# ubc-vision/DiffuseSG

Hardware: NVIDIA B200
Metric: sampled scene graphs/sec (higher is better)
Workload: dtype bf16

## Files before the change

### diffusesg_b200/build_native.py

```python
from __future__ import annotations

import os
import subprocess
import sys
from concurrent.futures import ThreadPoolExecutor

HERE = os.path.dirname(os.path.abspath(__file__))
CSRC = os.path.join(HERE, "csrc")
LIB_DIR = os.path.join(HERE, "lib")
LIB_PATH = os.path.join(LIB_DIR, "libdsg_b200.so")
SOURCES = ["gemm.cu", "mlp.cu", "blocktail.cu", "blockhead.cu", "projln.cu", "attention.cu", "attention_tc.cu", "rowops.cu", "edm.cu", "train.cu", "backward.cu", "pack.cu", "model.cu"]
HEADERS = ["common.cuh", "kernels.h", os.path.join("..", "..", "include", "dsg_b200.h")]
NVCC_FLAGS = ["-gencode", "arch=compute_100a,code=sm_100a", "-lineinfo", "-O3", "-std=c++17",
              "-Xcompiler", "-fPIC", "-Xcompiler", "-fvisibility=hidden", "--expt-relaxed-constexpr"]


def _nvcc() -> str:
    for cand in (os.environ.get("NVCC"), "/usr/local/cuda/bin/nvcc", "nvcc"):
        if cand and (os.path.isabs(cand) and os.path.exists(cand) or not os.path.isabs(cand)):
            return cand
    raise RuntimeError("nvcc not found")


def _stale(target: str, deps) -> bool:
    if not os.path.exists(target):
        return True
    t = os.path.getmtime(target)
    return any(os.path.getmtime(d) > t for d in deps)


def build(force: bool = False, verbose: bool = False) -> str:
    os.makedirs(LIB_DIR, exist_ok=True)
    hdrs = [os.path.normpath(os.path.join(CSRC, h)) for h in HEADERS]
    objs, jobs = [], []
    for src in SOURCES:
        s = os.path.join(CSRC, src)
        o = os.path.join(LIB_DIR, src.replace(".cu", ".o"))
        objs.append(o)
        if force or _stale(o, [s] + hdrs):
            jobs.append([_nvcc(), *NVCC_FLAGS, *(["-Xptxas", "-v"] if verbose else []), "-c", s, "-o", o])

    def run(cmd):
        r = subprocess.run(cmd, capture_output=True, text=True)
        if r.returncode != 0:
            raise RuntimeError("nvcc failed: %s\n%s\n%s" % (" ".join(cmd), r.stdout, r.stderr))
        return r.stderr

    with ThreadPoolExecutor(max_workers=6) as ex:
        for out in ex.map(run, jobs):
            if verbose and out:
                print(out)
    if force or jobs or _stale(LIB_PATH, objs):
        run([_nvcc(), "-shared", "-o", LIB_PATH, *objs, "-lcudart"])
    return LIB_PATH


if __name__ == "__main__":
    print(build(force="--force" in sys.argv, verbose="-v" in sys.argv))
```

### diffusesg_b200/csrc/blocktail.cu

```cuda
#include "common.cuh"
#include "kernels.h"

namespace dsg {
namespace {

constexpr int kTailThreads = 19 * 32;
constexpr float kTailLnEps = 1e-5f;

template <int C>
struct TailCfg {
  static constexpr int HID = 4 * C;
  static constexpr int HC = 128;
  static constexpr int NCH = HID / HC;
  static constexpr int KBN = C / 32;
  static constexpr int A_KB = 128 * 64;
  static constexpr int A_BYTES = KBN * A_KB;
  static constexpr int W1_KB = HC * 64;
  static constexpr int W1_SLOT = KBN * W1_KB;
  static constexpr int WP_KB = C * 64;
  static constexpr int W2_KB = C * 128;
  static constexpr int W2_SLOT = (HC / 64) * W2_KB;
  static constexpr int S1 = 2, S2 = 2;
  static constexpr int XB = C / 32;
  static constexpr int X_BYTES = XB * 16384;
// ... 472 lines not shown
        return;
      }
      if (tl > 0) mbar_wait(out_free, (tl - 1) & 1);
#pragma unroll
      for (int i = 0; i < G::CW; i += 4)
        *reinterpret_cast<float4*>(sXo + ((c0 + i) >> 5) * 16384 + r_t * 128 + ((((((c0 + i) & 31) >> 2)) ^ (r_t & 7)) << 4)) =
            make_float4(__uint_as_float(v[i]), __uint_as_float(v[i + 1]), __uint_as_float(v[i + 2]), __uint_as_float(v[i + 3]));
      fence_proxy_async_smem();
      __syncwarp();
      if (lane == 0) mbar_arrive(out_ready);
    };

    auto phase_g = [&](int g) {
      const int b = g & 1, j = g % G::NCH;
      mbar_wait(&acc1_full[b], (g >> 1) & 1);
      tcgen05_fence_after();
#pragma unroll
      for (int h = 0; h < 2; ++h) {
        const int col = cg * 32 + h * 16;
        uint32_t r[16];
        tmem_ld_32x16(t_lane + b * G::HC + col, r);
        tmem_ld_wait();
        uint32_t hp[8];
#pragma unroll
        for (int k = 0; k < 16; k += 4) {
          const float4 bb = *reinterpret_cast<const float4*>(&sB1[j * G::HC + col + k]);
          hp[k >> 1] = gelu_bias_bf16x2(r[k], r[k + 1], bb.x, bb.y);
          hp[(k >> 1) + 1] = gelu_bias_bf16x2(r[k + 2], r[k + 3], bb.z, bb.w);
        }
        tmem_st_32x8(t_lane + b * G::HC + col, hp);
      }
      tmem_st_wait();
      tcgen05_fence_before();
      __syncwarp();
      if (lane == 0) mbar_arrive(&h_full[b]);
    };

    if (my_tiles > 0) phase_p(0);
    for (int tl = 0; tl < my_tiles; ++tl) {
      const int g0 = tl * G::NCH;
      phase_g(g0);
      if (tl > 0) phase_o(tl - 1);
#pragma unroll 1
      for (int j = 1; j < G::NCH - 1; ++j) phase_g(g0 + j);
      if (tl + 1 < my_tiles) {
        mbar_wait(&acc1_full[(g0 + G::NCH - 1) & 1], ((g0 + G::NCH - 1) >> 1) & 1);
        phase_p(tl + 1);
      }
      phase_g(g0 + G::NCH - 1);
    }
    if (my_tiles > 0) phase_o(my_tiles - 1);
  }

  tcgen05_fence_before();
  __syncthreads();
  tcgen05_fence_after();
  if (warp == kMmaWarp) tmem_dealloc<512>(tmem_base);
}

template <int C>
int launch_c(const CUtensorMap* tmAtt, const CUtensorMap* tmWp, const CUtensorMap* tmW1, const CUtensorMap* tmW2,
             const CUtensorMap* tmX, const CUtensorMap* tmY, const TailParams& p, cudaStream_t st) {
  static PerDeviceOnce configured;
  if (configured.first()) {
    DSG_CUDA_CHECK(cudaFuncSetAttribute(block_tail_kernel<C, false>, cudaFuncAttributeMaxDynamicSharedMemorySize,
                                        TailCfg<C>::SMEM_BYTES));
    DSG_CUDA_CHECK(cudaFuncSetAttribute(block_tail_kernel<C, true>, cudaFuncAttributeMaxDynamicSharedMemorySize,
                                        TailCfg<C>::SMEM_BYTES));
  }
  const int sms = device_sm_count();
  const int tiles = (p.M + 127) / 128;
  if (tmY != nullptr)
    block_tail_kernel<C, true><<<tiles < sms ? tiles : sms, kTailThreads, TailCfg<C>::SMEM_BYTES, st>>>(
        *tmAtt, *tmWp, *tmW1, *tmW2, *tmX, *tmY, p);
  else
    block_tail_kernel<C, false><<<tiles < sms ? tiles : sms, kTailThreads, TailCfg<C>::SMEM_BYTES, st>>>(
        *tmAtt, *tmWp, *tmW1, *tmW2, *tmX, *tmX, p);
  DSG_LAUNCH_CHECK();
  return DSG_OK;
}

}

bool block_tail_supported(int C) { return C == 96; }

int launch_block_tail(const CUtensorMap* tmAtt, const CUtensorMap* tmWp, const CUtensorMap* tmW1,
                      const CUtensorMap* tmW2, const CUtensorMap* tmX, const float* bp, const float* gamma,
                      const float* beta, const float* b1, const float* b2, float* x, long long rows, int C,
                      cudaStream_t st, const CUtensorMap* tmY, const float* gamma_f, const float* beta_f) {
  DSG_REQUIRE(block_tail_supported(C) && rows > 0 && rows < 2147483647LL, "block_tail: C=%d rows=%lld", C, rows);
  DSG_REQUIRE((tmY == nullptr) == (gamma_f == nullptr) && (tmY == nullptr) == (beta_f == nullptr),
              "block_tail: the fused final LayerNorm needs its output map, gamma and beta together");
  TailParams p{bp, gamma, beta, b1, b2, x, gamma_f, beta_f, static_cast<int>(rows)};
  return launch_c<96>(tmAtt, tmWp, tmW1, tmW2, tmX, tmY, p, st);
}

}
```

### diffusesg_b200/csrc/kernels.h

```cpp
#pragma once

#include <cuda.h>
#include <cuda_bf16.h>
#include <cuda_runtime.h>
#include <stdint.h>

namespace dsg {

typedef __nv_bfloat16 bf16;

enum GemmEpi : int {
  EPI_BF16 = 0,
  EPI_GELU_BF16 = 1,
  EPI_RES_F32 = 2,
  EPI_F32 = 3,
  EPI_ADJ_HEAD = 4,
};

struct GemmParams {
  int M, N, K;
  const float* bias;
  const float* res;
  void* out;
  int ldo;
  int bn;
  int ksplit;
  int scale_rows;
  float row_scale;
  const float* w2t;
  const float* b2;
  int c_e;
  int n_img;
  const uint8_t* flags;
  const float* x_adj;
  const float* c_skip;
  const float* c_out;
  const int* perm;
  int side;
};

int make_tmap_bf16(CUtensorMap* map, const void* base, int64_t rows, int64_t cols, int box_rows);
int make_tmap_out(CUtensorMap* map, const void* base, int64_t rows, int64_t cols, int epi);

int launch_wgrad(const void* dy, const void* x, float* dw, long long tokens, int n_out, int x_cols, int out_cols, int ksplit,
                 int scale_rows, float row_scale, cudaStream_t st);

int gemm_block_n(int N);
int gemm_choose_bn(long long rows, int N, int K, int epi, bool pair);
bool gemm_use_pair(long long rows, int K, int epi);
int launch_gemm(const CUtensorMap* tmA, const CUtensorMap* tmW, const CUtensorMap* tmO, int epi, const GemmParams& p,
                cudaStream_t st, bool pair = false);

bool fused_mlp_supported(int C);
int fused_mlp_w1_box_rows(int C);
int launch_fused_mlp(const CUtensorMap* tmY, const CUtensorMap* tmW1, const CUtensorMap* tmW2, const CUtensorMap* tmX,
                     const float* b1, const float* b2, long long rows, int C, cudaStream_t st);

int make_tmap_2d(CUtensorMap* map, const void* base, int64_t rows, int64_t cols, int elem_bytes, int box_cols,
                 int box_rows);
bool block_tail_supported(int C);
int launch_block_tail(const CUtensorMap* tmAtt, const CUtensorMap* tmWp, const CUtensorMap* tmW1,
                      const CUtensorMap* tmW2, const CUtensorMap* tmX, const float* bp, const float* gamma,
                      const float* beta, const float* b1, const float* b2, float* x, long long rows, int C,
                      cudaStream_t st, const CUtensorMap* tmY = nullptr,
                      const float* gamma_f = nullptr, const float* beta_f = nullptr);

bool proj_ln_supported(int C);
int launch_proj_ln(const CUtensorMap* tmA, const CUtensorMap* tmW, const float* bias, const float* gamma, const float* beta,
                   float* x, bf16* y, long long rows, int C, cudaStream_t st);

bool block_head_supported(int C);
int launch_block_head(const CUtensorMap* tmXin, const CUtensorMap* tmXout, const CUtensorMap* tmW, const CUtensorMap* tmQ,
                      const float* film, int film_ld, int cond_uniform, int tokens_per_sample, const float* gamma,
                      const float* beta, const float* bqkv, long long rows, int C, cudaStream_t st);

int make_tmap_3d_bf16(CUtensorMap* map, const void* base, int64_t d0, int64_t d1, int64_t d2, int64_t s1, int64_t s2, int b0,
                      int b1, int b2);
bool window_attention_tc_supported(int batch, int res, int window, int shift, int heads);
int launch_window_attention_tc(const bf16* qkv, const float* bias, bf16* out, int batch, int res, int shift, int heads,
                               cudaStream_t st);
int launch_window_attention_tc_groups(const bf16* qkv, const float* bias, bf16* out, int n_groups, const int* counts,
                                      const int* res, const long long* tok_off, int heads, cudaStream_t st);
bool window_attention_quad_supported(int batch, int res, int window, int shift, int heads);
int launch_window_attention_quad(const bf16* qkv, const float* bias, bf16* out, int batch, int res, int window, int shift,
                                 int heads, cudaStream_t st);
int check_mask_canonical(const float* mask, int res, int window, int shift, cudaStream_t st, int* canonical);
bool window_attention_w16_supported(int batch, int res, int window, int shift, int heads);
int launch_window_attention_w16(const bf16* qkv, const float* bias, bf16* out, int batch, int res, int shift, int heads,
                                cudaStream_t st);
int check_bias_toeplitz(const float* bias, int heads, int window, cudaStream_t st, int* toeplitz);
enum { ATTN_MASK_CANONICAL = 1, ATTN_BIAS_TOEPLITZ = 2 };
int launch_window_attention(const bf16* qkv, const float* bias, const float* mask, bf16* out, int batch, int res,
                            int window, int shift, int heads, cudaStream_t st, int canonical = 0);

int launch_film_ln(const float* x_in, float* x_out, bf16* y, const float* film, int film_ld, int film_off,
                   int cond_uniform, const float* gamma, const float* beta, int batch, int tokens_per_sample,
                   int C, cudaStream_t st, const int* src_rows = nullptr);
int launch_ln(const float* x, bf16* y, const float* gamma, const float* beta, int64_t rows, int C, cudaStream_t st);
int launch_merge_ln(const float* x, bf16* y, const float* gamma, const float* beta, int batch, int res, int C,
                    cudaStream_t st);
int launch_concat_bf16(const float* x, const float* skip, bf16* y, int64_t rows, int C, cudaStream_t st,
                       const int* skip_rows = nullptr);
int launch_breakup_ln(const float* t, bf16* y, const float* g1, const float* b1, const float* g2, const float* b2,
                      int batch, int res, int D, cudaStream_t st);

int launch_cond(const float* noise_labels, long long label_stride, int n_cond, const float* w0, const float* b0, const float* w1,
                const float* b1, const float* w_film, const float* b_film, int film_total, float* emb0, float* emb1,
                float* emb, float* film, int embed, cudaStream_t st);

int launch_precond_coef(const float* sigmas, int sigma_stride, float* coef, int batch, cudaStream_t st);

int launch_node_proj(const float* node, const float* sc_node, const float* in_scale, const float* w_rc,
                     float* rc, int batch, int n, int c_n, int self_cond, int embed, cudaStream_t st);
int launch_patch_embed(const float* adj, const float* sc_adj, const float* in_scale, const uint8_t* flags,
                       const float* rc, const float* w_adj, const float* bias, const float* gamma,
                       const float* beta, const float* film, int film_ld, int film_off, int cond_uniform,
                       float* x0, int batch, int n, int c_e, int self_cond, int embed, cudaStream_t st,
                       const int* perm = nullptr, int side = 0);
int launch_node_head(const bf16* rep, const uint8_t* flags, const float* fold_t, const float* fold_b, const float* w1t,
                     const float* b1, const float* w2t, const float* b2, const float* x_node, const float* c_skip, const float* c_out,
                     float* out_node, int batch, int n, int c_n, int embed, cudaStream_t st, const int* tok0 = nullptr,
                     const int* width = nullptr, float* scratch = nullptr);

bool row_compaction_supported(int C_merge, int D_breakup);
int launch_breakup_ln_compact(const float* t, bf16* y, const float* g1, const float* b1, const float* g2, const float* b2,
                              int batch, int res, int D, const int* tok0, const int* width, int sh, cudaStream_t st,
                              const int* src_perm = nullptr);


int launch_edm_pre_step(const float* adj, const float* node, const float* eps_adj, const float* eps_node,
                        const uint8_t* flags, float noise_coef, float* adj_hat, float* node_hat, int batch,
                        int c_e, int n, int c_n, cudaStream_t st);
int launch_edm_pre_step_philox(const float* adj, const float* node, const uint8_t* flags, float noise_coef,
                               unsigned long long seed, unsigned long long offset_adj, int grid_adj,
                               unsigned long long offset_node, int grid_node, const void* dev_params, float* adj_hat,
                               float* node_hat, int batch, int c_e, int n, int c_n, cudaStream_t st);
int launch_edm_post_step(const float* adj_hat, const float* node_hat, const float* d1_adj, const float* d1_node,
                         const float* d2_adj, const float* d2_node, const uint8_t* flags, float inv_t_hat,
                         float h, float inv_t_prime, const void* dev_params, float* adj_next, float* node_next, int batch,
                         int c_e, int n, int c_n, cudaStream_t st);
int launch_edm_step_advance(const void* table, void* cur, int* counter, cudaStream_t st);
int launch_edm_final_decode(const float* adj_hat, const float* node_hat, const float* d1_adj, const float* d1_node,
                            const uint8_t* flags, float inv_t_hat, float h, const void* dev_params, float* adj_next,
                            float* node_next, int32_t* adj_cls, int32_t* node_cls, float* bbox, int num_adj_type,
                            int num_node_type, int batch, int c_e, int n, int c_n, cudaStream_t st);
int launch_mask_scale(const float* adj, const float* node, const uint8_t* flags, float scale, float* adj_out,
                      float* node_out, int batch, int c_e, int n, int c_n, cudaStream_t st);

// ... 25 lines not shown
```

### diffusesg_b200/csrc/model.cu

```cuda
#include <cstdarg>
#include <cstdio>
#include <cstdlib>
#include <cstring>
#include <map>
#include <string>
#include <tuple>
#include <vector>

#include "../../include/dsg_b200.h"
#include "common.cuh"
#include "kernels.h"

namespace dsg {

static thread_local char g_err[1024] = "";
static unsigned long long g_launches = 0;
static int g_stop_after = -1;

void set_last_error(const char* fmt, ...) {
  va_list ap;
  va_start(ap, fmt);
  vsnprintf(g_err, sizeof(g_err), fmt, ap);
  va_end(ap);
}
// ... 436 lines not shown
  p.M = static_cast<int>(rows); p.N = W.N; p.K = W.K;
  p.bias = bias; p.res = res; p.out = out; p.ldo = W.N;
  const double mn = static_cast<double>(rows) * W.N;
  const double out_bytes = epi == EPI_ADJ_HEAD ? static_cast<double>(rows) * (extra ? extra->c_e : 0) * 4
                                               : mn * ((epi == EPI_BF16 || epi == EPI_GELU_BF16) ? 2 : 4);
  char label[56];
  snprintf(label, sizeof(label), "gemm_n%d_k%d_epi%d", W.N, W.K, epi);
  ProfScope ps(g_prof_pass, PC_GEMM, 2.0 * mn * W.K,
               static_cast<double>(rows) * W.K * 2 + static_cast<double>(W.N) * W.K * 2 + out_bytes +
                   (epi == EPI_RES_F32 ? mn * 4 : 0), st, label, rows, W.K);
  const bool pair = gemm_use_pair(rows, W.K, epi);
  p.bn = gemm_choose_bn(rows, W.N, W.K, epi, pair);
  if (p.bn == 256) return launch_gemm(&it->second, pair ? &W.tmap256_half : &W.tmap256, tmo, epi, p, st, pair);
  return launch_gemm(&it->second, pair ? &W.tmap_half : &W.tmap, tmo, epi, p, st, pair);
}

#define DSG_TRY(expr)        \
  do {                       \
    int _rc = (expr);        \
    if (_rc) return _rc;     \
  } while (0)

#define DSG_TRY_P(cls, flops, bytes, expr)                                    \
  do {                                                                        \
    ProfScope _ps(g_prof_pass, cls, flops, bytes, st, #expr);                 \
    int _rc = (expr);                                                         \
    if (_rc) return _rc;                                                      \
  } while (0)

int run_block(dsg_model* m, const Block& b, const Workspace& w, const float* x_in, int batch, int cond_uniform,
              cudaStream_t st, bool fuse_final_ln = false, bool* fused_final_ln = nullptr, const Compact* cp = nullptr,
              const int* x_in_rows = nullptr) {
  const int C = b.dim;
  const int L = b.res * b.res;
  const long long rows = cp != nullptr ? cp->tokens(b.stage) : static_cast<long long>(batch) * L;
  const std::string& p = b.prefix;
  const double rc = static_cast<double>(rows) * C;
  auto tmap = [&](const void* ptr, int key, auto make) -> const CUtensorMap* {
    auto k = std::make_tuple(ptr, rows, key);
    auto it = m->a_maps.find(k);
    if (it == m->a_maps.end()) {
      CUtensorMap tm;
      if (make(&tm)) return nullptr;
      it = m->a_maps.emplace(k, tm).first;
    }
    return &it->second;
  };
  DSG_REQUIRE(x_in_rows == nullptr || (x_in != w.X && !block_head_supported(C)), "run_block: layout-changing input at C = %d", C);
  if (m->use_head && block_head_supported(C)) {
    const CUtensorMap* ti = tmap(x_in, -(C * 8 + EPI_RES_F32), [&](CUtensorMap* t) { return make_tmap_out(t, x_in, rows, C, EPI_RES_F32); });
    const CUtensorMap* to = tmap(w.X, -(C * 8 + EPI_RES_F32), [&](CUtensorMap* t) { return make_tmap_out(t, w.X, rows, C, EPI_RES_F32); });
    const CUtensorMap* tq = tmap(w.QKV, -(3 * C * 8 + EPI_BF16), [&](CUtensorMap* t) { return make_tmap_out(t, w.QKV, rows, 3 * C, EPI_BF16); });
    if (ti == nullptr || to == nullptr || tq == nullptr) return DSG_ERR_CUDA;
    DSG_TRY_P(PC_MLP, 6.0 * rc * C, rc * 14,
              launch_block_head(ti, to, &b.head_w, tq, w.film + b.film_off, m->film_total, cond_uniform, L,
                                m->f32(p + ".norm1.weight"), m->f32(p + ".norm1.bias"), m->at<float>(b.qkv_bias_off), rows,
                                C, st));
  } else {
    DSG_TRY_P(PC_ROW, 0, rc * 10, launch_film_ln(x_in, w.X, w.Y, w.film, m->film_total, b.film_off, cond_uniform,
                                                 m->f32(p + ".norm1.weight"), m->f32(p + ".norm1.bias"),
                                                 cp != nullptr ? 1 : batch, cp != nullptr ? static_cast<int>(rows) : L, C, st,
                                                 x_in_rows));
    DSG_TRY(gemm(m, w.Y, rows, b.qkv, EPI_BF16, m->at<float>(b.qkv_bias_off), nullptr, w.QKV, st));
  }
  const float* mask = b.shift > 0 ? m->f32(p + ".attn_mask") : nullptr;
  if (cp != nullptr && b.window == 8 && cp->K <= 4) {
    int res_k[4];
    long long tok_k[4];
    for (int k = 0; k < cp->K; ++k) { res_k[k] = cp->side[k] >> b.stage; tok_k[k] = cp->at(k, b.stage); }
    DSG_TRY_P(PC_ATTN, 4.0 * rc * b.window * b.window, rc * 8,
              launch_window_attention_tc_groups(w.QKV, m->at<float>(b.attn_bias_off), w.ATT, cp->K, cp->count, res_k, tok_k, b.heads, st));
  } else if (cp != nullptr) {
    for (int k = 0; k < cp->K; ++k) {
      const long long t0 = cp->at(k, b.stage), tk = cp->at(k + 1, b.stage) - t0;
      DSG_TRY_P(PC_ATTN, 4.0 * tk * C * b.window * b.window, static_cast<double>(tk) * C * 8,
                launch_window_attention(w.QKV + t0 * 3 * C, m->at<float>(b.attn_bias_off), nullptr, w.ATT + t0 * C, cp->count[k],
                                        cp->side[k] >> b.stage, b.window, 0, b.heads, st, b.mask_canonical));
    }
  } else {
    DSG_TRY_P(PC_ATTN, 4.0 * rc * b.window * b.window, rc * 8,
              launch_window_attention(w.QKV, m->at<float>(b.attn_bias_off), mask, w.ATT, batch, b.res, b.window, b.shift,
                                      b.heads, st, b.mask_canonical));
  }
  if (m->use_tail && block_tail_supported(C)) {
    const CUtensorMap* ta = tmap(w.ATT, 100000 + C, [&](CUtensorMap* t) { return make_tmap_2d(t, w.ATT, rows, C, 2, 32, 128); });
    const CUtensorMap* tx = tmap(w.X, -(C * 8 + EPI_RES_F32), [&](CUtensorMap* t) { return make_tmap_out(t, w.X, rows, C, EPI_RES_F32); });
    if (ta == nullptr || tx == nullptr) return DSG_ERR_CUDA;
    const CUtensorMap* ty = nullptr;
    if (fuse_final_ln) {
      ty = tmap(w.Y, -(C * 8 + EPI_BF16), [&](CUtensorMap* t) { return make_tmap_out(t, w.Y, rows, C, EPI_BF16); });
      if (ty == nullptr) return DSG_ERR_CUDA;
      if (fused_final_ln) *fused_final_ln = true;
    }
    DSG_TRY_P(PC_MLP, 18.0 * rc * C, rc * (fuse_final_ln ? 8 : 10),
              launch_block_tail(ta, &b.tail_wp, &b.tail_w1, &b.mlp_w2, tx, m->f32(p + ".attn.proj.bias"),
                                m->f32(p + ".norm2.weight"), m->f32(p + ".norm2.bias"), m->f32(p + ".mlp.fc1.bias"),
                                m->f32(p + ".mlp.fc2.bias"), w.X, rows, C, st, ty,
                                fuse_final_ln ? m->f32("norm.weight") : nullptr,
                                fuse_final_ln ? m->f32("norm.bias") : nullptr));
    return DSG_OK;
  }
  if (C == 384) {
    const CUtensorMap* ta = tmap(w.ATT, C, [&](CUtensorMap* t) { return make_tmap_bf16(t, w.ATT, rows, C, 128); });
    if (ta == nullptr) return DSG_ERR_CUDA;
    DSG_TRY_P(PC_MLP, 2.0 * rc * C, rc * 12,
              launch_proj_ln(ta, &b.proj.tmap, m->f32(p + ".attn.proj.bias"), m->f32(p + ".norm2.weight"),
                             m->f32(p + ".norm2.bias"), w.X, w.Y, rows, C, st));
  } else {
    DSG_TRY(gemm(m, w.ATT, rows, b.proj, EPI_RES_F32, m->f32(p + ".attn.proj.bias"), w.X, w.X, st));
    DSG_TRY_P(PC_ROW, 0, rc * 6, launch_ln(w.X, w.Y, m->f32(p + ".norm2.weight"), m->f32(p + ".norm2.bias"), rows, C, st));
  }
  if (m->use_fused_mlp && fused_mlp_supported(C)) {
    const CUtensorMap* ty = tmap(w.Y, C, [&](CUtensorMap* t) { return make_tmap_bf16(t, w.Y, rows, C, 128); });
    const CUtensorMap* tx = tmap(w.X, -(C * 8 + EPI_RES_F32), [&](CUtensorMap* t) { return make_tmap_out(t, w.X, rows, C, EPI_RES_F32); });
    if (ty == nullptr || tx == nullptr) return DSG_ERR_CUDA;
    DSG_TRY_P(PC_MLP, 16.0 * rc * C, rc * 10,
              launch_fused_mlp(ty, &b.mlp_w1, &b.mlp_w2, tx, m->f32(p + ".mlp.fc1.bias"), m->f32(p + ".mlp.fc2.bias"), rows,
                               C, st));
    return DSG_OK;
  }
  DSG_TRY(gemm(m, w.Y, rows, b.fc1, EPI_GELU_BF16, m->f32(p + ".mlp.fc1.bias"), nullptr, w.H, st));
  DSG_TRY(gemm(m, w.H, rows, b.fc2, EPI_RES_F32, m->f32(p + ".mlp.fc2.bias"), w.X, w.X, st));
  return DSG_OK;
}

}

extern "C" {

int dsg_abi_version(void) { return DSG_ABI_VERSION; }
void dsg_debug_set_smem_poison(unsigned pattern, int enable) {
  g_smem_poison = pattern;
  g_smem_poison_on = enable != 0;
}
const char* dsg_last_error(void) { return g_err; }
uint64_t dsg_launch_count(void) { return __atomic_load_n(&g_launches, __ATOMIC_RELAXED); }

int dsg_model_create(const dsg_config* cfg, dsg_model** out) {
  DSG_REQUIRE(cfg != nullptr && out != nullptr, "dsg_model_create: null argument");
  dsg_model* m = new dsg_model();
  m->cfg = *cfg;
  const char* no_fuse = getenv("DSG_NO_FUSED_MLP");
  m->use_fused_mlp = !(no_fuse != nullptr && no_fuse[0] == '1');
  const char* no_tail = getenv("DSG_NO_TAIL");
  m->use_tail = !(no_tail != nullptr && no_tail[0] == '1');
  const char* no_head = getenv("DSG_NO_HEAD");
  m->use_head = !(no_head != nullptr && no_head[0] == '1');
  const int rc = build(m);
  if (rc) { delete m; return rc; }
  *out = m;
  return DSG_OK;
}

void dsg_model_destroy(dsg_model* m) { delete m; }

size_t dsg_model_arena_bytes(const dsg_model* m) { return m ? m->arena_bytes : 0; }

int dsg_model_bind_arena(dsg_model* m, void* arena, size_t bytes) {
  DSG_REQUIRE(m != nullptr && arena != nullptr, "bind_arena: null argument");
  if (bytes < m->arena_bytes || (reinterpret_cast<uintptr_t>(arena) & (kAlign - 1)) != 0) {
    set_last_error("bind_arena: need %zu bytes aligned to %zu, got %zu at %p", m->arena_bytes, kAlign, bytes, arena);
    return DSG_ERR_WORKSPACE;
  }
  m->arena = static_cast<uint8_t*>(arena);
  m->finalized = false;
  for (TensorSpec& t : m->tensors) t.loaded = false;
  return DSG_OK;
}

int dsg_model_num_tensors(const dsg_model* m) { return m ? static_cast<int>(m->tensors.size()) : 0; }

int dsg_model_tensor_info(const dsg_model* m, int i, const char** key, int64_t* numel, int32_t* dtype) {
  DSG_REQUIRE(m != nullptr && i >= 0 && i < static_cast<int>(m->tensors.size()), "tensor_info: index %d", i);
  if (key) *key = m->tensors[i].key.c_str();
  if (numel) *numel = m->tensors[i].numel;
  if (dtype) *dtype = m->tensors[i].dtype;
  return DSG_OK;
}

int dsg_model_set_tensor(dsg_model* m, const char* key, const void* src, int64_t bytes, int src_is_host,
                         dsg_stream_t stream) {
  DSG_REQUIRE(m != nullptr && key != nullptr && src != nullptr, "set_tensor: null argument");
  if (m->arena == nullptr) { set_last_error("set_tensor: no arena bound"); return DSG_ERR_STATE; }
  auto it = m->index.find(key);
  if (it == m->index.end()) { set_last_error("set_tensor: unknown key '%s'", key); return DSG_ERR_UNKNOWN_KEY; }
  TensorSpec& t = m->tensors[it->second];
  DSG_REQUIRE(static_cast<size_t>(bytes) == t.bytes(), "set_tensor: '%s' expects %zu bytes, got %lld", key, t.bytes(),
              static_cast<long long>(bytes));
  DSG_CUDA_CHECK(cudaMemcpyAsync(m->arena + t.offset, src, t.bytes(),
                                 src_is_host ? cudaMemcpyHostToDevice : cudaMemcpyDeviceToDevice,
                                 static_cast<cudaStream_t>(stream)));
  t.loaded = true;
  m->finalized = false;
  return DSG_OK;
}

int dsg_model_tensor_differs(const dsg_model* m, const char* key, const void* src, int64_t bytes, int32_t* flag,
                             dsg_stream_t stream) {
  DSG_REQUIRE(m != nullptr && key != nullptr && src != nullptr && flag != nullptr, "tensor_differs: null argument");
  if (m->arena == nullptr) { set_last_error("tensor_differs: no arena bound"); return DSG_ERR_STATE; }
  auto it = m->index.find(key);
  if (it == m->index.end()) { set_last_error("tensor_differs: unknown key '%s'", key); return DSG_ERR_UNKNOWN_KEY; }
  const TensorSpec& t = m->tensors[it->second];
  DSG_REQUIRE(static_cast<size_t>(bytes) == t.bytes() && (reinterpret_cast<uintptr_t>(src) & 3) == 0,
              "tensor_differs: '%s' expects %zu bytes (4-byte aligned), got %lld", key, t.bytes(), static_cast<long long>(bytes));
  return launch_compare_words(m->arena + t.offset, src, static_cast<int64_t>(t.bytes() / 4), flag,
                              static_cast<cudaStream_t>(stream));
}

int dsg_model_finalize(dsg_model* m, dsg_stream_t stream) {
  DSG_REQUIRE(m != nullptr, "finalize: null model");
  if (m->arena == nullptr) { set_last_error("finalize: no arena bound"); return DSG_ERR_STATE; }
  for (const TensorSpec& t : m->tensors)
    if (!t.loaded) { set_last_error("finalize: tensor '%s' was never set", t.key.c_str()); return DSG_ERR_STATE; }
  cudaStream_t st = static_cast<cudaStream_t>(stream);
  const float qscale = 0.17677669529663687f;
  for (Block& b : m->blocks) {
    const int C = b.dim, T = b.window * b.window;
    const std::string& p = b.prefix;
    DSG_TRY(pack_weight(m, b.qkv, p + ".attn.qkv.weight", st, static_cast<int64_t>(C) * C, qscale));
    DSG_TRY(launch_scale_copy(m->f32(p + ".attn.qkv.bias"), m->at<float>(b.qkv_bias_off), 3 * C, C, qscale, st));
    DSG_TRY(pack_weight(m, b.proj, p + ".attn.proj.weight", st));
    DSG_TRY(pack_weight(m, b.fc1, p + ".mlp.fc1.weight", st));
    DSG_TRY(pack_weight(m, b.fc2, p + ".mlp.fc2.weight", st));
    if (fused_mlp_supported(C)) {
      DSG_TRY(make_tmap_bf16(&b.mlp_w1, m->arena + b.fc1.offset, 4 * C, C, fused_mlp_w1_box_rows(C)));
      DSG_TRY(make_tmap_bf16(&b.mlp_w2, m->arena + b.fc2.offset, C, 4 * C, C));
    }
    if (block_head_supported(C)) DSG_TRY(make_tmap_2d(&b.head_w, m->arena + b.qkv.offset, 3 * C, C, 2, 32, C));
    if (block_tail_supported(C)) {
      DSG_TRY(make_tmap_2d(&b.tail_wp, m->arena + b.proj.offset, C, C, 2, 32, C));
      DSG_TRY(make_tmap_2d(&b.tail_w1, m->arena + b.fc1.offset, 4 * C, C, 2, 32, 128));
    }
    const TensorSpec& idx = m->tensors[m->index[p + ".attn.relative_position_index"]];
    DSG_TRY(launch_bias_expand(m->f32(p + ".attn.relative_position_bias_table"),
                               reinterpret_cast<const int64_t*>(m->arena + idx.offset), m->at<float>(b.attn_bias_off), T,
                               b.heads, (2 * b.window - 1) * (2 * b.window - 1), st));
    b.mask_canonical = 0;
    const bool w16 = window_attention_w16_supported(1, b.res, b.window, b.shift, b.heads);
    if (b.shift > 0 && (w16 || window_attention_quad_supported(1, b.res, b.window, b.shift, b.heads))) {
      int ok = 0;
      DSG_TRY(check_mask_canonical(m->f32(p + ".attn_mask"), b.res, b.window, b.shift, st, &ok));
      if (ok) b.mask_canonical |= ATTN_MASK_CANONICAL;
    }
    if (w16) {
      int ok = 0;
      DSG_TRY(check_bias_toeplitz(m->at<float>(b.attn_bias_off), b.heads, b.window, st, &ok));
      if (ok) b.mask_canonical |= ATTN_BIAS_TOEPLITZ;
    }
  }
  for (Merge& g : m->merges) DSG_TRY(pack_weight(m, g.reduction, g.prefix + ".reduction.weight", st));
  for (Breakup& u : m->breakups) {
    DSG_TRY(pack_weight(m, u.pre, u.prefix + ".pre_linear.weight", st));
    DSG_TRY(pack_weight(m, u.post, u.prefix + ".post_linear.weight", st));
  }
  const int E = m->E;
  const float* wp = m->f32("patch_embed.proj.weight");
  DSG_TRY(launch_transpose(wp, m->at<float>(m->w_adj_off), E, m->cin, 0, m->planes_adj, E, st));
  DSG_TRY(launch_transpose(wp, m->at<float>(m->w_rc_off), E, m->cin, m->planes_adj, m->planes_node, E, st));
  DSG_TRY(launch_transpose(wp, m->at<float>(m->w_rc_off) + static_cast<size_t>(m->planes_node) * E, E, m->cin,
                           m->planes_adj + m->planes_node, m->planes_node, E, st));
  float* t1 = m->at<float>(m->fold_t1_off);
  float* ff = m->at<float>(m->fold_f_off);
  float* tv = m->at<float>(m->fold_tv_off);
  DSG_TRY(launch_small_mm(m->f32("read_out.1.weight"), m->f32("read_out.0.weight"), t1, E, 1, st));
  DSG_TRY(launch_small_mm(m->f32("read_out.2.weight"), t1, ff, E, 0, st));
  DSG_TRY(launch_small_mv(m->f32("read_out.1.weight"), m->f32("read_out.0.bias"), m->f32("read_out.1.bias"), tv, E, st));
  DSG_TRY(launch_small_mv(m->f32("read_out.2.weight"), tv, m->f32("read_out.2.bias"), m->at<float>(m->fold_b_off), E, st));
  DSG_TRY(launch_small_mm(m->f32("readout_adj_mlp.fc1.weight"), ff, t1, E, 0, st));
  DSG_TRY(launch_pack_bf16(t1, m->at<bf16>(m->adj_fc1.offset), static_cast<int64_t>(E) * E, 0, 1.f, st));
  DSG_TRY(make_tmap_bf16(&m->adj_fc1.tmap, m->arena + m->adj_fc1.offset, E, E, gemm_block_n(E)));
  DSG_TRY(launch_small_mv(m->f32("readout_adj_mlp.fc1.weight"), m->at<float>(m->fold_b_off),
                          m->f32("readout_adj_mlp.fc1.bias"), m->at<float>(m->adj_b1_off), E, st));
  DSG_TRY(launch_transpose(ff, m->at<float>(m->fold_ft_off), E, E, 0, E, E, st));
  DSG_CUDA_CHECK(cudaMemsetAsync(m->at<float>(m->adj_w2t_off), 0, static_cast<size_t>(E) * 8 * 4, st));
  DSG_CUDA_CHECK(cudaMemsetAsync(m->at<float>(m->adj_b2_off), 0, 8 * 4, st));
  DSG_TRY(launch_transpose(m->f32("readout_adj_mlp.fc2.weight"), m->at<float>(m->adj_w2t_off), m->cfg.c_e, E, 0, E, 8, st));
  DSG_CUDA_CHECK(cudaMemcpyAsync(m->at<float>(m->adj_b2_off), m->f32("readout_adj_mlp.fc2.bias"), m->cfg.c_e * 4,
                                 cudaMemcpyDeviceToDevice, st));
  DSG_TRY(launch_transpose(m->f32("readout_node_mlp.fc1.weight"), m->at<float>(m->node_w1t_off), E, E, 0, E, E, st));
  DSG_TRY(launch_transpose(m->f32("readout_node_mlp.fc2.weight"), m->at<float>(m->node_w2t_off), m->cfg.c_n, E, 0, E,
                           m->cfg.c_n, st));
  m->finalized = true;
  return DSG_OK;
}

int dsg_model_skip_info(const dsg_model* m, int32_t* stages, int32_t* granule) {
  DSG_REQUIRE(m != nullptr && stages != nullptr && granule != nullptr, "skip_info: null argument");
  *stages = m->skip_stages;
  *granule = m->skip_granule;
  return DSG_OK;
}

int dsg_model_skip_info2(const dsg_model* m, int32_t* granule2) {
  DSG_REQUIRE(m != nullptr && granule2 != nullptr, "skip_info2: null argument");
  *granule2 = m->skip2_granule;
  return DSG_OK;
}

size_t dsg_workspace_bytes(const dsg_model* m, int batch, int n_cond) {
  if (m == nullptr || batch <= 0 || n_cond <= 0) return 0;
  return carve(m, batch, n_cond, nullptr).bytes;
}

int dsg_denoiser_forward(dsg_model* m, const dsg_forward_args* a, dsg_stream_t stream) {
  DSG_REQUIRE(m != nullptr && a != nullptr, "forward: null argument");
  DSG_REQUIRE(a->struct_size == sizeof(dsg_forward_args), "forward: dsg_forward_args size %u, library expects %zu",
              a->struct_size, sizeof(dsg_forward_args));
  if (!m->finalized) { set_last_error("forward: dsg_model_finalize has not been called since the last weight update"); return DSG_ERR_STATE; }
  DSG_REQUIRE(a->batch > 0 && (a->n_cond == 1 || a->n_cond == a->batch), "forward: batch %d n_cond %d", a->batch, a->n_cond);
  DSG_REQUIRE(a->mode == 0 || a->mode == 1, "forward: mode %d", a->mode);
  DSG_REQUIRE(a->adj && a->node && a->flags && a->noise && a->out_adj && a->out_node, "forward: null tensor");
  DSG_REQUIRE((reinterpret_cast<uintptr_t>(a->flags) & 3) == 0, "forward: node_flags must be 4-byte aligned");
// ... 490 lines not shown
```

Measured before the change: 66.73.

## Add fused cluster-pair block tail kernel for C=384 Swin blocks

Adds a new tcgen05 kernel for the 384-channel blocks that runs on a 2-CTA cluster. It fuses the attention projection, residual add, LayerNorm, fc1 with GELU, fc2 and the second residual into one persistent kernel, with warp-specialised TMA, MMA and epilogue warps and 256-row paired tiles. The goal is to remove the separate GEMM and LayerNorm launches and their intermediate global-memory round trips for the deepest stage. The cost is a large, complex pipeline of mbarriers with tight shared-memory and TMEM budgets.

Measured after the change: 70.73, median of 6. +6.0%, better.

```diff
diff --git a/diffusesg_b200/build_native.py b/diffusesg_b200/build_native.py
--- a/diffusesg_b200/build_native.py
+++ b/diffusesg_b200/build_native.py
@@ -9,7 +9,7 @@
 CSRC = os.path.join(HERE, "csrc")
 LIB_DIR = os.path.join(HERE, "lib")
 LIB_PATH = os.path.join(LIB_DIR, "libdsg_b200.so")
-SOURCES = ["gemm.cu", "mlp.cu", "blocktail.cu", "blockhead.cu", "projln.cu", "attention.cu", "attention_tc.cu", "rowops.cu", "edm.cu", "train.cu", "backward.cu", "pack.cu", "model.cu"]
+SOURCES = ["gemm.cu", "mlp.cu", "blocktail.cu", "blocktail384.cu", "blockhead.cu", "projln.cu", "attention.cu", "attention_tc.cu", "rowops.cu", "edm.cu", "train.cu", "backward.cu", "pack.cu", "model.cu"]
 HEADERS = ["common.cuh", "kernels.h", os.path.join("..", "..", "include", "dsg_b200.h")]
 NVCC_FLAGS = ["-gencode", "arch=compute_100a,code=sm_100a", "-lineinfo", "-O3", "-std=c++17",
               "-Xcompiler", "-fPIC", "-Xcompiler", "-fvisibility=hidden", "--expt-relaxed-constexpr"]
diff --git a/diffusesg_b200/csrc/blocktail.cu b/diffusesg_b200/csrc/blocktail.cu
--- a/diffusesg_b200/csrc/blocktail.cu
+++ b/diffusesg_b200/csrc/blocktail.cu
@@ -578,13 +578,13 @@
 
 }
 
-bool block_tail_supported(int C) { return C == 96; }
+bool block_tail_supported(int C) { return C == 96 || C == 384; }
 
 int launch_block_tail(const CUtensorMap* tmAtt, const CUtensorMap* tmWp, const CUtensorMap* tmW1,
                       const CUtensorMap* tmW2, const CUtensorMap* tmX, const float* bp, const float* gamma,
                       const float* beta, const float* b1, const float* b2, float* x, long long rows, int C,
                       cudaStream_t st, const CUtensorMap* tmY, const float* gamma_f, const float* beta_f) {
-  DSG_REQUIRE(block_tail_supported(C) && rows > 0 && rows < 2147483647LL, "block_tail: C=%d rows=%lld", C, rows);
+  DSG_REQUIRE(C == 96 && rows > 0 && rows < 2147483647LL, "block_tail: C=%d rows=%lld", C, rows);
   DSG_REQUIRE((tmY == nullptr) == (gamma_f == nullptr) && (tmY == nullptr) == (beta_f == nullptr),
               "block_tail: the fused final LayerNorm needs its output map, gamma and beta together");
   TailParams p{bp, gamma, beta, b1, b2, x, gamma_f, beta_f, static_cast<int>(rows)};
diff --git a/diffusesg_b200/csrc/blocktail384.cu b/diffusesg_b200/csrc/blocktail384.cu
--- /dev/null
+++ b/diffusesg_b200/csrc/blocktail384.cu
@@ -0,0 +1,474 @@
+#include "common.cuh"
+#include "kernels.h"
+
+namespace dsg {
+namespace {
+
+constexpr int kC = 384;
+constexpr int kHid = 4 * kC;
+constexpr int kHC = 128;
+constexpr int kNCH = kHid / kHC;
+constexpr int kKB = kC / 64;
+constexpr int kKbBytes = 128 * 128;
+constexpr int kAyBytes = kKB * kKbBytes;
+constexpr int kHBytes = 2 * kKbBytes;
+constexpr int kStage = 24576;
+constexpr int kHalfN = 96 * 128;
+constexpr int kStages = 3;
+constexpr int kXSlots = kAyBytes / 16384;
+constexpr int kParFloats = kHid + 4 * kC;
+constexpr int kPartBytes = 4 * 128 * 8;
+constexpr int kWorkers = 16;
+constexpr int kThreads = (kWorkers + 3) * 32;
+constexpr int kSmemBytes = 1024 + kAyBytes + kHBytes + kStages * kStage + kParFloats * 4 + kPartBytes + 256;
+constexpr float kLnEps = 1e-5f;
+static_assert(kSmemBytes <= 227 * 1024, "block tail 384: shared memory budget");
+static_assert(kWorkers * 2048 <= kHBytes, "O staging (2 KB per worker warp) must fit the H buffer");
+
+struct Tail384Params {
+  const float* bp;
+  const float* gamma;
+  const float* beta;
+  const float* b1;
+  const float* b2;
+  int M;
+};
+
+DSG_DEVICE void tmem_ld_32x8(uint32_t taddr, uint32_t* r) {
+  asm volatile("tcgen05.ld.sync.aligned.32x32b.x8.b32 {%0, %1, %2, %3, %4, %5, %6, %7}, [%8];"
+               : "=r"(r[0]), "=r"(r[1]), "=r"(r[2]), "=r"(r[3]), "=r"(r[4]), "=r"(r[5]), "=r"(r[6]), "=r"(r[7])
+               : "r"(taddr)
+               : "memory");
+}
+DSG_DEVICE void tmem_st_32x8(uint32_t taddr, const uint32_t* r) {
+  asm volatile("tcgen05.st.sync.aligned.32x32b.x8.b32 [%0], {%1, %2, %3, %4, %5, %6, %7, %8};"
+               ::"r"(taddr), "r"(r[0]), "r"(r[1]), "r"(r[2]), "r"(r[3]), "r"(r[4]), "r"(r[5]), "r"(r[6]), "r"(r[7])
+               : "memory");
+}
+DSG_DEVICE void tmem_st_wait() { asm volatile("tcgen05.wait::st.sync.aligned;" ::: "memory"); }
+
+DSG_DEVICE uint32_t sw128(int r, int u) { return static_cast<uint32_t>(r * 128 + (((u ^ r) & 7) << 4)); }
+
+__global__ void __launch_bounds__(kThreads, 1)
+block_tail_pair_kernel(const __grid_constant__ CUtensorMap tmAtt, const __grid_constant__ CUtensorMap tmWp,
+                       const __grid_constant__ CUtensorMap tmW1, const __grid_constant__ CUtensorMap tmW2,
+                       const __grid_constant__ CUtensorMap tmX, const __grid_constant__ CUtensorMap tmXo,
+                       const Tail384Params p) {
+  extern __shared__ uint8_t smem_raw[];
+  uint8_t* smem = smem_raw + ((1024u - (smem_u32(smem_raw) & 1023u)) & 1023u);
+  uint8_t* sAY = smem;
+  uint8_t* sH = sAY + kAyBytes;
+  uint8_t* sW = sH + kHBytes;
+  float* sB1 = reinterpret_cast<float*>(sW + kStages * kStage);
+  float* sBp = sB1 + kHid;
+  float* sB2 = sBp + kC;
+  float* sGam = sB2 + kC;
+  float* sBet = sGam + kC;
+  float2* sPart = reinterpret_cast<float2*>(sBet + kC);
+  uint64_t* bars = reinterpret_cast<uint64_t*>(reinterpret_cast<uint8_t*>(sPart) + kPartBytes);
+  uint64_t* w_full = bars;
+  uint64_t* w_empty = w_full + kStages;
+  uint64_t* x_full = w_empty + kStages;
+  uint64_t* x_empty = x_full + kXSlots;
+  uint64_t* att_full = x_empty + kXSlots;
+  uint64_t* att_empty = att_full + 1;
+  uint64_t* proj_full = att_full + 2;
+  uint64_t* y_ready = att_full + 3;
+  uint64_t* acc1_full = att_full + 4;
+  uint64_t* acc1_empty = att_full + 5;
+  uint64_t* h_full = att_full + 6;
+  uint64_t* h_empty = att_full + 7;
+  uint64_t* out_full = att_full + 8;
+  uint64_t* acc_empty = att_full + 9;
+  uint32_t* tmem_slot = reinterpret_cast<uint32_t*>(att_full + 10);
+
+  const int warp = uniform_warp_id();
+  const int lane = threadIdx.x & 31;
+  constexpr int kTmaWarp = kWorkers, kMmaWarp = kWorkers + 1, kXWarp = kWorkers + 2;
+  const uint32_t rank = cluster_ctarank();
+  const int pair = blockIdx.x >> 1, npairs = gridDim.x >> 1;
+  const int num_tiles = (p.M + 255) / 256;
+  const int my_tiles = (num_tiles > pair) ? (num_tiles - pair + npairs - 1) / npairs : 0;
+  auto row0_of = [&](int tl) { return (pair + tl * npairs) * 256 + static_cast<int>(rank) * 128; };
+
+  if (warp == kTmaWarp && lane == 0) {
+    tma_prefetch_desc(&tmAtt);
+    tma_prefetch_desc(&tmWp);
+    tma_prefetch_desc(&tmW1);
+    tma_prefetch_desc(&tmW2);
+    tma_prefetch_desc(&tmX);
+    tma_prefetch_desc(&tmXo);
+    for (int s = 0; s < kStages; ++s) { mbar_init(&w_full[s], 1); mbar_init(&w_empty[s], 1); }
+    for (int s = 0; s < kXSlots; ++s) { mbar_init(&x_full[s], 1); mbar_init(&x_empty[s], kWorkers); }
+    mbar_init(att_full, 1);
+    mbar_init(att_empty, 1);
+    mbar_init(proj_full, 1);
+    mbar_init(y_ready, 2 * kWorkers);
+    mbar_init(acc1_full, 1);
+    mbar_init(acc1_empty, 2 * kWorkers);
+    mbar_init(h_full, 2 * kWorkers);
+    mbar_init(h_empty, 1);
+    mbar_init(out_full, 1);
+    mbar_init(acc_empty, 2 * kWorkers);
+    fence_barrier_init();
+  }
+  if (warp == kMmaWarp) tmem_alloc_pair<512>(tmem_slot);
+  for (int i = threadIdx.x; i < kHid; i += kThreads) sB1[i] = p.b1[i];
+  for (int i = threadIdx.x; i < kC; i += kThreads) {
+    sBp[i] = p.bp[i];
+    sB2[i] = p.b2[i];
+    sGam[i] = p.gamma[i];
+    sBet[i] = p.beta[i];
+  }
+  tcgen05_fence_before();
+  __syncthreads();
+  cluster_sync_all();
+  tcgen05_fence_after();
+  const uint32_t tmem_base = uniform_u32(*tmem_slot);
+  constexpr uint32_t kAcc1 = kC;
+
+  if (warp == kTmaWarp) {
+    if (elect_one()) {
+      int s = 0;
+      uint32_t ph = 0;
+      auto stage = [&]() -> uint8_t* {
+        mbar_wait(&w_empty[s], ph ^ 1);
+        if (rank == 0) mbar_expect_tx(&w_full[s], 2 * kStage);
+        return sW + s * kStage;
+      };
+      auto advance = [&]() { if (++s == kStages) { s = 0; ph ^= 1; } };
+      auto load_w1 = [&](int g, int half) {
+        uint8_t* dst = stage();
+        const uint32_t bar = mapa_u32(&w_full[s], 0);
+        for (int j = 0; j < 3; ++j)
+          tma_load_2d_pair(dst + j * 8192, &tmW1, bar, (3 * half + j) * 64, g * kHC + static_cast<int>(rank) * 64);
+        advance();
+      };
+      auto load_w2 = [&](int g, int kb) {
+        uint8_t* dst = stage();
+        const uint32_t bar = mapa_u32(&w_full[s], 0);
+        for (int n = 0; n < 2; ++n)
+          tma_load_2d_pair(dst + n * kHalfN, &tmW2, bar, g * kHC + kb * 64, n * 192 + static_cast<int>(rank) * 96);
+        advance();
+      };
+      const uint32_t att_bar = mapa_u32(att_full, 0);
+      for (int tl = 0; tl < my_tiles; ++tl) {
+        mbar_wait(att_empty, (tl & 1) ^ 1);
+        if (rank == 0) mbar_expect_tx(att_full, 2 * kAyBytes);
+        for (int kb = 0; kb < kKB; ++kb) tma_load_2d_pair(sAY + kb * kKbBytes, &tmAtt, att_bar, kb * 64, row0_of(tl));
+        for (int kb = 0; kb < kKB; ++kb) {
+          uint8_t* dst = stage();
+          const uint32_t bar = mapa_u32(&w_full[s], 0);
+          for (int n = 0; n < 2; ++n)
+            tma_load_2d_pair(dst + n * kHalfN, &tmWp, bar, kb * 64, n * 192 + static_cast<int>(rank) * 96);
+          advance();
+        }
+        load_w1(0, 0);
+        load_w1(0, 1);
+        for (int g = 0; g < kNCH; ++g) {
+          if (g + 1 < kNCH) { load_w1(g + 1, 0); load_w1(g + 1, 1); }
+          load_w2(g, 0);
+          load_w2(g, 1);
+        }
+      }
+    }
+  } else if (warp == kMmaWarp && rank == 0) {
+    constexpr uint32_t idesc_n = umma_idesc_bf16_pair(192);
+    constexpr uint32_t idesc_h = umma_idesc_bf16_pair(kHC);
+    int s = 0;
+    uint32_t ph = 0;
+    auto wait_stage = [&]() { mbar_wait(&w_full[s], ph); tcgen05_fence_after(); };
+    auto advance = [&]() { if (++s == kStages) { s = 0; ph ^= 1; } };
+    auto fc1 = [&](int n, int g) {
+      if (n > 0) { mbar_wait(acc1_empty, (n - 1) & 1); tcgen05_fence_after(); }
+      for (int half = 0; half < 2; ++half) {
+        wait_stage();
+        if (elect_one()) {
+          for (int j = 0; j < 3; ++j) {
+            const int kb = 3 * half + j;
+            const uint64_t da = umma_desc_sw128(smem_u32(sAY + kb * kKbBytes));
+            const uint64_t db = umma_desc_sw128(smem_u32(sW + s * kStage + j * 8192));
+            for (int k = 0; k < 4; ++k) umma_bf16_ss_pair(tmem_base + kAcc1, da + 2 * k, db + 2 * k, idesc_h, (kb | k) != 0);
+          }
+          umma_commit_pair(&w_empty[s]);
+          if (half == 1) {
+            umma_commit_pair(acc1_full);
+            if (g == kNCH - 1) umma_commit_pair(att_empty);
+          }
+        }
+        __syncwarp();
+        advance();
+      }
+    };
+    auto fc2 = [&](int n, int g) {
+      mbar_wait(h_full, n & 1);
+      tcgen05_fence_after();
+      for (int kb = 0; kb < 2; ++kb) {
+        wait_stage();
+        if (elect_one()) {
+          const uint64_t da = umma_desc_sw128(smem_u32(sH + kb * kKbBytes));
+          for (int h = 0; h < 2; ++h) {
+            const uint64_t db = umma_desc_sw128(smem_u32(sW + s * kStage + h * kHalfN));
+            for (int k = 0; k < 4; ++k) umma_bf16_ss_pair(tmem_base + h * 192, da + 2 * k, db + 2 * k, idesc_n, 1u);
+          }
+          umma_commit_pair(&w_empty[s]);
+          if (kb == 1) {
+            umma_commit_pair(h_empty);
+            if (g == kNCH - 1) umma_commit_pair(out_full);
+          }
+        }
+        __syncwarp();
+        advance();
+      }
+    };
+    for (int tl = 0; tl < my_tiles; ++tl) {
+      mbar_wait(att_full, tl & 1);
+      mbar_wait(acc_empty, (tl & 1) ^ 1);
+      tcgen05_fence_after();
+      for (int kb = 0; kb < kKB; ++kb) {
+        wait_stage();
+        if (elect_one()) {
+          const uint64_t da = umma_desc_sw128(smem_u32(sAY + kb * kKbBytes));
+          for (int h = 0; h < 2; ++h) {
+            const uint64_t db = umma_desc_sw128(smem_u32(sW + s * kStage + h * kHalfN));
+            for (int k = 0; k < 4; ++k) umma_bf16_ss_pair(tmem_base + h * 192, da + 2 * k, db + 2 * k, idesc_n, (kb | k) != 0);
+          }
+          umma_commit_pair(&w_empty[s]);
+          if (kb == kKB - 1) umma_commit_pair(proj_full);
+        }
+        __syncwarp();
+        advance();
+      }
+      mbar_wait(y_ready, tl & 1);
+      tcgen05_fence_after();
+      const int n0 = tl * kNCH;
+      fc1(n0, 0);
+      for (int g = 0; g < kNCH; ++g) {
+        if (g + 1 < kNCH) fc1(n0 + g + 1, g + 1);
+        fc2(n0 + g, g);
+      }
+    }
+  } else if (warp == kMmaWarp) {
+  } else if (warp == kXWarp) {
+    if (elect_one()) {
+      auto prefetch = [&](int tl) {
+        const int r0 = row0_of(tl);
+        for (int c = 0; c < kC / 32; ++c)
+          asm volatile("cp.async.bulk.prefetch.tensor.2d.L2.global.tile [%0, {%1, %2}];"
+                       ::"l"(reinterpret_cast<uint64_t>(&tmX)), "r"(c * 32), "r"(r0) : "memory");
+        for (int kb = 0; kb < kKB; ++kb)
+          asm volatile("cp.async.bulk.prefetch.tensor.2d.L2.global.tile [%0, {%1, %2}];"
+                       ::"l"(reinterpret_cast<uint64_t>(&tmAtt)), "r"(kb * 64), "r"(r0) : "memory");
+      };
+      for (int tl = 0; tl < my_tiles; ++tl) {
+        mbar_wait(proj_full, tl & 1);
+        for (int c = 0; c < kC / 32; ++c) {
+          const int sl = c % kXSlots;
+          const uint32_t use = tl * 2 + c / kXSlots;
+          mbar_wait(&x_empty[sl], (use & 1) ^ 1);
+          mbar_expect_tx(&x_full[sl], 16384);
+          tma_load_2d(sAY + sl * 16384, &tmX, &x_full[sl], c * 32, row0_of(tl));
+        }
+        if (tl + 1 < my_tiles) prefetch(tl + 1);
+      }
+    }
+  } else {
+    const int q = warp & 3;
+    const int cg = warp >> 2;
+    const int r = q * 32 + lane;
+    const uint32_t t_lane = tmem_base + (static_cast<uint32_t>(q * 32) << 16);
+    const uint32_t y_ready_l = mapa_u32(y_ready, 0), acc1_empty_l = mapa_u32(acc1_empty, 0);
+    const uint32_t h_full_l = mapa_u32(h_full, 0), acc_empty_l = mapa_u32(acc_empty, 0);
+    uint8_t* stg = sH + warp * 2048;
+
+    for (int tl = 0; tl < my_tiles; ++tl) {
+      mbar_wait(proj_full, tl & 1);
+      tcgen05_fence_after();
+      float pivot = 0.f;
+      f32x2 npiv = f2_splat(0.f), s1 = f2_splat(0.f), s2 = f2_splat(0.f);
+#pragma unroll 1
+      for (int i = 0; i < kC / 32; ++i) {
+        const int sl = i % kXSlots;
+        const uint32_t use = tl * 2 + i / kXSlots;
+        const int c0 = 32 * i + 8 * cg;
+        uint32_t v[8];
+        tmem_ld_32x8(t_lane + c0, v);
+        mbar_wait(&x_full[sl], use & 1);
+        const uint8_t* xs = sAY + sl * 16384;
+        const float4 x0 = *reinterpret_cast<const float4*>(xs + sw128(r, 2 * cg));
+        const float4 x1 = *reinterpret_cast<const float4*>(xs + sw128(r, 2 * cg + 1));
+        if (i == 0) {
+          pivot = *reinterpret_cast<const float*>(xs + sw128(r, 0));
+          npiv = f2_splat(-pivot);
+        }
+        __syncwarp();
+        if (lane == 0) mbar_arrive(&x_empty[sl]);
+        tmem_ld_wait();
+        const float xv[8] = {x0.x, x0.y, x0.z, x0.w, x1.x, x1.y, x1.z, x1.w};
+        uint32_t o[8];
+#pragma unroll
+        for (int j = 0; j < 8; j += 2) {
+          const f32x2 a = f2_add(f2_add(f2_pack(__uint_as_float(v[j]), __uint_as_float(v[j + 1])),
+                                        f2_pack(sBp[c0 + j], sBp[c0 + j + 1])),
+                                 f2_pack(xv[j], xv[j + 1]));
+          const f32x2 d = f2_add(a, npiv);
+          s1 = f2_add(s1, d);
+          s2 = f2_fma(d, d, s2);
+          float lo, hi;
+          f2_unpack(a, lo, hi);
+          o[j] = __float_as_uint(lo);
+          o[j + 1] = __float_as_uint(hi);
+        }
+        tmem_st_32x8(t_lane + c0, o);
+      }
+      {
+        float s1a, s1b, s2a, s2b;
+        f2_unpack(s1, s1a, s1b);
+        f2_unpack(s2, s2a, s2b);
+        sPart[cg * 128 + r] = make_float2(s1a + s1b, s2a + s2b);
+      }
+      tmem_st_wait();
+      asm volatile("bar.sync 1, %0;" ::"n"(kWorkers * 32) : "memory");
+      float t1 = 0.f, t2 = 0.f;
+#pragma unroll
+      for (int k = 0; k < 4; ++k) {
+        const float2 pp = sPart[k * 128 + r];
+        t1 += pp.x;
+        t2 += pp.y;
+      }
+      const float dm = t1 * (1.0f / kC);
+      const float rstd = rsqrtf(fmaxf(t2 * (1.0f / kC) - dm * dm, 0.f) + kLnEps);
+      const f32x2 rs2 = f2_splat(rstd), nmr = f2_splat(-(pivot + dm) * rstd);
+#pragma unroll 1
+      for (int i = 0; i < kC / 32; ++i) {
+        const int c0 = 32 * i + 8 * cg;
+        uint32_t v[8];
+        tmem_ld_32x8(t_lane + c0, v);
+        tmem_ld_wait();
+        uint32_t yk[4], w[8];
+#pragma unroll
+        for (int j = 0; j < 8; j += 2) {
+          const f32x2 a = f2_pack(__uint_as_float(v[j]), __uint_as_float(v[j + 1]));
+          yk[j >> 1] = pack_bf16x2(f2_fma(f2_fma(a, rs2, nmr), f2_pack(sGam[c0 + j], sGam[c0 + j + 1]),
+                                          f2_pack(sBet[c0 + j], sBet[c0 + j + 1])));
+          float lo, hi;
+          f2_unpack(f2_add(a, f2_pack(sB2[c0 + j], sB2[c0 + j + 1])), lo, hi);
+          w[j] = __float_as_uint(lo);
+          w[j + 1] = __float_as_uint(hi);
+        }
+        *reinterpret_cast<uint4*>(sAY + (c0 >> 6) * kKbBytes + sw128(r, (c0 & 63) >> 3)) = make_uint4(yk[0], yk[1], yk[2], yk[3]);
+        tmem_st_32x8(t_lane + c0, w);
+      }
+      tmem_st_wait();
+      fence_proxy_async_smem();
+      tcgen05_fence_before();
+      __syncwarp();
+      if (lane == 0) mbar_arrive_cluster(y_ready_l);
+
+#pragma unroll 1
+      for (int g = 0; g < kNCH; ++g) {
+        const int n = tl * kNCH + g;
+        mbar_wait(acc1_full, n & 1);
+        tcgen05_fence_after();
+        uint32_t ra[16], rb[16];
+        tmem_ld_32x16(t_lane + kAcc1 + cg * 32, ra);
+        tmem_ld_32x16(t_lane + kAcc1 + cg * 32 + 16, rb);
+        tmem_ld_wait();
+        tcgen05_fence_before();
+        __syncwarp();
+        if (lane == 0) mbar_arrive_cluster(acc1_empty_l);
+        const float* b1 = sB1 + g * kHC + cg * 32;
+        uint32_t hp[16];
+#pragma unroll
+        for (int k = 0; k < 16; k += 2) {
+          hp[k >> 1] = gelu_bias_bf16x2(ra[k], ra[k + 1], b1[k], b1[k + 1]);
+          hp[8 + (k >> 1)] = gelu_bias_bf16x2(rb[k], rb[k + 1], b1[16 + k], b1[16 + k + 1]);
+        }
+        mbar_wait(h_empty, (n & 1) ^ 1);
+        uint8_t* hrow = sH + (cg >> 1) * kKbBytes;
+#pragma unroll
+        for (int u = 0; u < 4; ++u)
+          *reinterpret_cast<uint4*>(hrow + sw128(r, (cg & 1) * 4 + u)) =
+              make_uint4(hp[4 * u], hp[4 * u + 1], hp[4 * u + 2], hp[4 * u + 3]);
+        fence_proxy_async_smem();
+        __syncwarp();
+        if (lane == 0) mbar_arrive_cluster(h_full_l);
+      }
+
+      mbar_wait(out_full, tl & 1);
+      tcgen05_fence_after();
+      const int orow = row0_of(tl) + q * 32;
+#pragma unroll 1
+      for (int i = 0; i < 6; ++i) {
+        const int col = cg * 96 + 16 * i;
+        uint32_t v[16];
+        tmem_ld_32x16(t_lane + col, v);
+        if (lane == 0) asm volatile("cp.async.bulk.wait_group.read 0;" ::: "memory");
+        __syncwarp();
+        tmem_ld_wait();
+        if (i == 5) {
+          tcgen05_fence_before();
+          __syncwarp();
+          if (lane == 0) mbar_arrive_cluster(acc_empty_l);
+        }
+#pragma unroll
+        for (int u = 0; u < 4; ++u)
+          *reinterpret_cast<float4*>(stg + lane * 64 + (((u ^ (lane >> 1)) & 3) << 4)) =
+              make_float4(__uint_as_float(v[4 * u]), __uint_as_float(v[4 * u + 1]), __uint_as_float(v[4 * u + 2]),
+                          __uint_as_float(v[4 * u + 3]));
+        fence_proxy_async_smem();
+        __syncwarp();
+        if (lane == 0) {
+          asm volatile("cp.async.bulk.tensor.2d.global.shared::cta.bulk_group [%0, {%2, %3}], [%1];"
+                       ::"l"(reinterpret_cast<uint64_t>(&tmXo)), "r"(smem_u32(stg)), "r"(col), "r"(orow)
+                       : "memory");
+          asm volatile("cp.async.bulk.commit_group;" ::: "memory");
+        }
+      }
+      if (lane == 0) asm volatile("cp.async.bulk.wait_group.read 0;" ::: "memory");
+      __syncwarp();
+    }
+    if (lane == 0) asm volatile("cp.async.bulk.wait_group 0;" ::: "memory");
+  }
+
+  tcgen05_fence_before();
+  __syncthreads();
+  cluster_sync_all();
+  tcgen05_fence_after();
+  if (warp == kMmaWarp) tmem_dealloc_pair<512>(tmem_base);
+}
+
+}
+
+int launch_block_tail_pair(const CUtensorMap* tmAtt, const CUtensorMap* tmWp, const CUtensorMap* tmW1,
+                           const CUtensorMap* tmW2, const CUtensorMap* tmX, const CUtensorMap* tmXo, const float* bp,
+                           const float* gamma, const float* beta, const float* b1, const float* b2, long long rows,
+                           int C, cudaStream_t st) {
+  DSG_REQUIRE(C == kC && rows > 0 && rows < 2147483647LL, "block_tail_pair: C=%d rows=%lld", C, rows);
+  DSG_REQUIRE(bp && gamma && beta && b1 && b2, "block_tail_pair: null parameter");
+  static PerDeviceOnce configured;
+  if (configured.first()) {
+    DSG_CUDA_CHECK(cudaFuncSetAttribute(block_tail_pair_kernel, cudaFuncAttributeMaxDynamicSharedMemorySize, kSmemBytes));
+  }
+  const Tail384Params p{bp, gamma, beta, b1, b2, static_cast<int>(rows)};
+  const int tiles = static_cast<int>((rows + 255) / 256);
+  const int max_pairs = device_sm_count() / 2;
+  const int pairs = tiles < max_pairs ? tiles : max_pairs;
+  cudaLaunchConfig_t cfg = {};
+  cfg.gridDim = dim3(2 * pairs);
+  cfg.blockDim = dim3(kThreads);
+  cfg.dynamicSmemBytes = kSmemBytes;
+  cfg.stream = st;
+  cudaLaunchAttribute attr[1];
+  attr[0].id = cudaLaunchAttributeClusterDimension;
+  attr[0].val.clusterDim.x = 2;
+  attr[0].val.clusterDim.y = 1;
+  attr[0].val.clusterDim.z = 1;
+  cfg.attrs = attr;
+  cfg.numAttrs = 1;
+  DSG_CUDA_CHECK(cudaLaunchKernelEx(&cfg, block_tail_pair_kernel, *tmAtt, *tmWp, *tmW1, *tmW2, *tmX, *tmXo, p));
+  DSG_LAUNCH_CHECK();
+  return DSG_OK;
+}
+
+}
diff --git a/diffusesg_b200/csrc/kernels.h b/diffusesg_b200/csrc/kernels.h
--- a/diffusesg_b200/csrc/kernels.h
+++ b/diffusesg_b200/csrc/kernels.h
@@ -64,6 +64,10 @@
                       const float* beta, const float* b1, const float* b2, float* x, long long rows, int C,
                       cudaStream_t st, const CUtensorMap* tmY = nullptr,
                       const float* gamma_f = nullptr, const float* beta_f = nullptr);
+int launch_block_tail_pair(const CUtensorMap* tmAtt, const CUtensorMap* tmWp, const CUtensorMap* tmW1,
+                           const CUtensorMap* tmW2, const CUtensorMap* tmX, const CUtensorMap* tmXo, const float* bp,
+                           const float* gamma, const float* beta, const float* b1, const float* b2, long long rows,
+                           int C, cudaStream_t st);
 
 bool proj_ln_supported(int C);
 int launch_proj_ln(const CUtensorMap* tmA, const CUtensorMap* tmW, const float* bias, const float* gamma, const float* beta,
diff --git a/diffusesg_b200/csrc/model.cu b/diffusesg_b200/csrc/model.cu
--- a/diffusesg_b200/csrc/model.cu
+++ b/diffusesg_b200/csrc/model.cu
@@ -542,6 +542,17 @@
               launch_window_attention(w.QKV, m->at<float>(b.attn_bias_off), mask, w.ATT, batch, b.res, b.window, b.shift,
                                       b.heads, st, b.mask_canonical));
   }
+  if (m->use_tail && block_tail_supported(C) && C == 384) {
+    const CUtensorMap* ta = tmap(w.ATT, C, [&](CUtensorMap* t) { return make_tmap_bf16(t, w.ATT, rows, C, 128); });
+    const CUtensorMap* tx = tmap(w.X, -(C * 8 + EPI_RES_F32), [&](CUtensorMap* t) { return make_tmap_out(t, w.X, rows, C, EPI_RES_F32); });
+    const CUtensorMap* to = tmap(w.X, 200000 + C, [&](CUtensorMap* t) { return make_tmap_2d(t, w.X, rows, C, 4, 16, 32); });
+    if (ta == nullptr || tx == nullptr || to == nullptr) return DSG_ERR_CUDA;
+    DSG_TRY_P(PC_MLP, 18.0 * rc * C, rc * 10,
+              launch_block_tail_pair(ta, &b.proj.tmap_half, &b.tail_w1, &b.fc2.tmap_half, tx, to,
+                                     m->f32(p + ".attn.proj.bias"), m->f32(p + ".norm2.weight"), m->f32(p + ".norm2.bias"),
+                                     m->f32(p + ".mlp.fc1.bias"), m->f32(p + ".mlp.fc2.bias"), rows, C, st));
+    return DSG_OK;
+  }
   if (m->use_tail && block_tail_supported(C)) {
     const CUtensorMap* ta = tmap(w.ATT, 100000 + C, [&](CUtensorMap* t) { return make_tmap_2d(t, w.ATT, rows, C, 2, 32, 128); });
     const CUtensorMap* tx = tmap(w.X, -(C * 8 + EPI_RES_F32), [&](CUtensorMap* t) { return make_tmap_out(t, w.X, rows, C, EPI_RES_F32); });
@@ -688,7 +699,9 @@
       DSG_TRY(make_tmap_bf16(&b.mlp_w2, m->arena + b.fc2.offset, C, 4 * C, C));
     }
     if (block_head_supported(C)) DSG_TRY(make_tmap_2d(&b.head_w, m->arena + b.qkv.offset, 3 * C, C, 2, 32, C));
-    if (block_tail_supported(C)) {
+    if (block_tail_supported(C) && C == 384) {
+      DSG_TRY(make_tmap_bf16(&b.tail_w1, m->arena + b.fc1.offset, 4 * C, C, 64));
+    } else if (block_tail_supported(C)) {
       DSG_TRY(make_tmap_2d(&b.tail_wp, m->arena + b.proj.offset, C, C, 2, 32, C));
       DSG_TRY(make_tmap_2d(&b.tail_w1, m->arena + b.fc1.offset, 4 * C, C, 2, 32, 128));
     }
```
